# afermg/aliby

Hardware: AMD Instinct MI355X
Metric: FOV tiles/sec (whole node) (higher is better)
Workload: dtype u16 pixels, f64 feature accumulators, f32 dynamics, bfloat16 U-Net

## Files before the change

### aliby_amd/csrc/nn_conv.hip

```cpp
#include "common.h"
#include "conv_launch.h"
#include "conv_mfma.h"

namespace {

struct ConvArgs {
  const uint4* in;
  const uint4* wpk;
  uint4* out;
  uint4* pool;
  const float* scale;
  const float* shift;
  const float* bias;
  const uint4* res;
  int shift_stride, res_up;
  int cs, coff;
  int ocs, ocoff;
  int N, H, W;
  int G;
  int tiles_x, tiles_y, ntiles;
  int order;
  const uint4* pin;
  const uint4* pwpk;
  int pcs;
  const float* hscale;
  const float* hshift;
  const float* hw;
  const float* hbias;
  float* hout;
  int hO;
  const uint4* wpk2;
  const float* scale2;
  const float* shift2;
  const float* bias2;
  int shift2_stride;
  const float* fx;
  const float* fw;
  const float* fscale;
  const float* fshift;
  int fcin;
  unsigned long long* trace;
};

#define CONV_STAMP(slot_)                                                                   \
  do {                                                                                      \
    if (a.trace && blockIdx.x == 0 && tid == 0 && stamp_tile < 16)                          \
      a.trace[stamp_tile * 8 + (slot_)] = __builtin_amdgcn_s_memtime();                     \
  } while (0)



template <int R>
__device__ __forceinline__ void conv_load_res(const ConvArgs& a, int n, int irow, int row0, int gx, int c0, uint4 (&rr)[R][2]) {
  const int RH = a.H >> a.res_up, RW = a.W >> a.res_up;
  const uint4* resN = a.res + (size_t)n * RH * RW * a.ocs + a.ocoff;
#pragma unroll
  for (int r = 0; r < R; ++r) {
    const int cy = min(row0 + r, a.H - 1), cx = min(gx, a.W - 1);
    const unsigned off = (unsigned)((((irow + cy) >> a.res_up) * RW + (cx >> a.res_up)) * a.ocs + (c0 >> 3));
    rr[r][0] = resN[off];
    rr[r][1] = resN[off + 1];
  }
}

template <int R>
__device__ __forceinline__ void conv_seed(f32x16_t (&acc)[R], const float4 (&b4)[4], const uint4 (&rr)[R][2], bool has_res) {
#pragma unroll
  for (int r = 0; r < R; ++r) {
    acc_seed(acc[r], b4);
    if (has_res) {
      const unsigned rw[8] = {rr[r][0].x, rr[r][0].y, rr[r][0].z, rr[r][0].w, rr[r][1].x, rr[r][1].y, rr[r][1].z, rr[r][1].w};
#pragma unroll
      for (int q = 0; q < 8; ++q) {
        acc[r][2 * q] += cv_bf2f(rw[q] & 0xffffu);
        acc[r][2 * q + 1] += cv_bf2f(rw[q] >> 16);
      }
    }
  }
}

template <int R, int KC, int DEPTH, int PLANE, int LW, bool LOW = false>
__device__ __forceinline__ void conv_mfma(const bf16x8_t* L, const bf16x8_t (&wfrag)[9 * KC], f32x16_t (&acc)[R], const bf16x8_t* L1 = nullptr) {
  constexpr int NF = (R + 2) * 3 * KC;
  bf16x8_t ring[DEPTH];
  auto frag = [&](int f) {
    const int ir = f / (3 * KC), dx = (f / KC) % 3;
    if constexpr (LOW) return (dx == 1 ? L1 : L)[2 * (f % KC) * PLANE + ((ir + 1) >> 1) * LW + (dx == 2)];
    else return L[2 * (f % KC) * PLANE + ir * LW + dx];
  };
#pragma unroll
  for (int f = 0; f < DEPTH - 1; ++f) ring[f] = frag(f);
  static_for<NF>([&](auto fc) {
    constexpr int f = decltype(fc)::value;
    if constexpr (f + DEPTH - 1 < NF) ring[(f + DEPTH - 1) % DEPTH] = frag(f + DEPTH - 1);
    constexpr int ir = f / (3 * KC), dx = (f / KC) % 3, kc = f % KC;
    static_for<3>([&](auto dc) {
      constexpr int dy = decltype(dc)::value, r = ir - dy;
      if constexpr (r >= 0 && r < R)
        acc[r] = __builtin_amdgcn_mfma_f32_32x32x16_bf16(wfrag[(dy * 3 + dx) * KC + kc], ring[f % DEPTH], acc[r], 0, 0, 0);
    });
    __builtin_amdgcn_sched_barrier(0);
  });
}

template <int R>
__device__ __forceinline__ void conv_store(const ConvArgs& a, int n, int irow, int row0, int gx, int c0, const f32x16_t (&acc)[R]) {
  if (gx >= a.W) return;
#pragma unroll
  for (int r = 0; r < R; ++r) {
    const int gy = row0 + r;
    if (gy >= a.H) continue;
    uint4* op = a.out + (size_t)n * a.H * a.W * a.ocs + a.ocoff + (unsigned)(((irow + gy) * a.W + gx) * a.ocs + (c0 >> 3));
    acc_pack16(acc[r], op[0], op[1]);
  }
}

struct HeadW { bf16x8_t w[2]; };

__device__ __forceinline__ HeadW head_weights(const float* hw, int hO, int lane) {
  HeadW h;
  const int hh = lane >> 5, o = conv_row_channel(lane & 31);
#pragma unroll
  for (int kc = 0; kc < 2; ++kc) {
    unsigned r4[4];
#pragma unroll
    for (int j2 = 0; j2 < 4; ++j2) {
      const int c = 16 * kc + 8 * hh + 2 * j2;
      r4[j2] = cv_pack2(o < hO ? hw[o * 32 + c] : 0.f, o < hO ? hw[o * 32 + c + 1] : 0.f);
    }
    h.w[kc] = __builtin_bit_cast(bf16x8_t, make_uint4(r4[0], r4[1], r4[2], r4[3]));
  }
  return h;
}

__device__ __forceinline__ f32x16_t head_apply(uint4 lo, uint4 hi, const float* sc, const float* sh, const HeadW& hw, int hh) {
  f32x2_t s2[4], h2[4];
  const float* sp = sc + 16 * hh;
  const float* hp = sh + 16 * hh;
#pragma unroll
  for (int k = 0; k < 4; ++k) { s2[k] = f32x2_t{sp[2 * k], sp[2 * k + 1]}; h2[k] = f32x2_t{hp[2 * k], hp[2 * k + 1]}; }
  const uint4 alo = conv_act8(lo, s2, h2, 0xffffffffu);
#pragma unroll
  for (int k = 0; k < 4; ++k) { s2[k] = f32x2_t{sp[8 + 2 * k], sp[8 + 2 * k + 1]}; h2[k] = f32x2_t{hp[8 + 2 * k], hp[8 + 2 * k + 1]}; }
  const uint4 ahi = conv_act8(hi, s2, h2, 0xffffffffu);
  const uint4 send = hh ? alo : ahi;
  const uint4 recv = make_uint4(__shfl_xor(send.x, 32), __shfl_xor(send.y, 32), __shfl_xor(send.z, 32), __shfl_xor(send.w, 32));
  const uint4 b0 = hh ? recv : alo, b1 = hh ? ahi : recv;
  f32x16_t y;
#pragma unroll
  for (int k = 0; k < 16; ++k) y[k] = 0.f;
  y = __builtin_amdgcn_mfma_f32_32x32x16_bf16(hw.w[0], __builtin_bit_cast(bf16x8_t, b0), y, 0, 0, 0);
  y = __builtin_amdgcn_mfma_f32_32x32x16_bf16(hw.w[1], __builtin_bit_cast(bf16x8_t, b1), y, 0, 0, 0);
  return y;
}

__device__ __forceinline__ f32x16_t head_from_acc(const f32x16_t& acc, const float* sc, const float* sh, const HeadW& hw, int hh) {
  return head_apply(acc_pack8(acc, 0), acc_pack8(acc, 1), sc, sh, hw, hh);
}

template <int CIN, int COUT, bool TALL = false, bool PACK = false, bool HEAD = false>
struct ConvCfg {
  static constexpr int KC = CIN / 16;
  static constexpr int NPL = CIN / 8;
  static constexpr int NCB = COUT / 32;
  static constexpr int R = (CIN >= 64 || HEAD) ? 2 : 4;
  static constexpr int PASSES = (PACK && COUT >= 128) ? 7 : ((CIN >= 64 && COUT >= 64) ? 2 : 1) * (TALL ? 2 : 1) * (HEAD ? 2 : 1);
  static constexpr int RG = 4 / NCB;
  static constexpr int TH = RG * R * PASSES, TW = 32, LH = TH + 2, LW = TW + 2 + (PACK ? 1 : 0);
  static constexpr int RAW = LH * LW;
  static constexpr int PLANE = NPL == 4 ? RAW + (10 - RAW % 8) % 8 : (RAW | 1);
  static constexpr int LDS_BYTES = NPL * PLANE * 16;
  static constexpr int PIX_PER_IT = 256 / NPL;
  static constexpr int ITERS = (RAW + PIX_PER_IT - 1) / PIX_PER_IT;
  static constexpr int C3_B32T = 1;
  static constexpr int C3_B64T = 4;
  static constexpr int NBATCH = (PACK && COUT >= 128) ? 3 : (CIN >= 64 ? ((TALL && COUT == 64) ? C3_B64T : 2) : (TALL ? C3_B32T : 1));
  static constexpr int BATCH = (ITERS + NBATCH - 1) / NBATCH;
  static constexpr int DEPTH = (CIN >= 64 && COUT >= 64) ? 4 : 6;
  static constexpr int DEPTH_POOL = (CIN >= 64 && COUT >= 64) ? 3 : 6;
};

template <int CIN, int COUT, bool UP, bool POOL, int PK, bool TALL, bool PACK = false, bool HEAD = false>
__global__ __launch_bounds__(256, 2) void k_conv3x3(ConvArgs a) {
  static_assert(!PACK || (!UP && PK == 0), "packed launches: plain input, no fused projection");
  static_assert(!HEAD || (COUT == 32 && !POOL && PK == 0 && !PACK), "the fused head is built for the 32-channel last unit");
  using cfg = ConvCfg<CIN, COUT, TALL, PACK, HEAD>;
  constexpr int PPLANE = (cfg::TH * cfg::TW) | 1;
  constexpr int KC = cfg::KC, NPL = cfg::NPL, NCB = cfg::NCB, R = cfg::R, TH = cfg::TH, TW = cfg::TW;
  constexpr int LW = cfg::LW, RAW = cfg::RAW, PLANE = cfg::PLANE, PASSES = cfg::PASSES;
  constexpr int PIX_PER_IT = cfg::PIX_PER_IT, ITERS = cfg::ITERS, BATCH = cfg::BATCH;
  extern __shared__ uint4 lds[];

  const int tid = threadIdx.x, lane = tid & 63, wave = tid >> 6;
  const int cb = wave % NCB, rg = wave / NCB;
  const int px = lane & 31, hh = lane >> 5;

  bf16x8_t wfrag[9 * KC];
  {
    const bf16x8_t* wp = reinterpret_cast<const bf16x8_t*>(a.wpk) + (size_t)cb * 9 * KC * 64 + lane;
#pragma unroll
    for (int i = 0; i < 9 * KC; ++i) wfrag[i] = wp[i * 64];
  }
  bf16x8_t pfrag[PK > 0 ? PK : 1];
  if constexpr (PK > 0) {
    const bf16x8_t* pp = reinterpret_cast<const bf16x8_t*>(a.pwpk) + (size_t)cb * PK * 64 + lane;
#pragma unroll
    for (int i = 0; i < PK; ++i) pfrag[i] = pp[i * 64];
  }
  uint4* const ldsP = lds + NPL * PLANE;
  __shared__ float4 sbias[COUT / 4];
  if (tid < COUT / 4) sbias[tid] = a.bias ? reinterpret_cast<const float4*>(a.bias)[tid] : make_float4(0.f, 0.f, 0.f, 0.f);
  __shared__ float hconst[HEAD ? 2 * 32 + 4 : 1];
  HeadW hwf;
  if constexpr (HEAD) {
    hwf = head_weights(a.hw, a.hO, lane);
    if (tid < 32) {
      hconst[tid] = a.hscale[tid];
      hconst[32 + tid] = a.hshift[tid];
      if (tid < 4) hconst[64 + tid] = tid < a.hO ? a.hbias[tid] : 0.f;
    }
  }
  const int pl = tid % NPL, pix0 = tid / NPL;
  const int ly0 = pix0 / LW, lx0 = pix0 - ly0 * LW;
  f32x2_t sc[4];
#pragma unroll
  for (int k = 0; k < 4; ++k) sc[k] = f32x2_t{a.scale[pl * 8 + 2 * k], a.scale[pl * 8 + 2 * k + 1]};

  const int IH = UP ? a.H >> 1 : a.H, IW = UP ? a.W >> 1 : a.W;
  const TileWalk walk = tile_walk(a.ntiles, a.order);

  for (int stamp_tile = 0; stamp_tile < walk.count; ++stamp_tile) {
    const int tile = walk.first + stamp_tile * walk.step;
    CONV_STAMP(0);
    const int tx = tile % a.tiles_x, tyn = tile / a.tiles_x;
    const int ty = tyn % a.tiles_y, n = tyn / a.tiles_y;
    const int y0 = ty * TH, x0 = tx * TW;
    int g0 = 0, cst = x0, kb = 1 << 20, nimg = n;
    if constexpr (PACK) {
      g0 = x0 / a.W;
      cst = x0 - g0 * a.W;
      kb = a.W - cst;
      nimg = n * a.G;
    }

    f32x2_t sh[4], sh1[PACK ? 4 : 1];
    {
      const float* sp = a.shift + (size_t)(nimg + g0) * a.shift_stride + pl * 8;
#pragma unroll
      for (int k = 0; k < 4; ++k) sh[k] = f32x2_t{sp[2 * k], sp[2 * k + 1]};
      if constexpr (PACK) {
        const float* sq = a.shift + (size_t)(nimg + min(g0 + 1, a.G - 1)) * a.shift_stride + pl * 8;
#pragma unroll
        for (int k = 0; k < 4; ++k) sh1[k] = f32x2_t{sq[2 * k], sq[2 * k + 1]};
      }
    }
    const int second = (PACK && px >= kb) ? 1 : 0;
    const int gx = PACK ? (second ? px - kb : cst + px) : x0 + px;
    const int irow = PACK ? (g0 + second) * a.H : 0;
    const int c0 = cb * 32 + hh * 16;
    uint4 rr[R][2];
    auto load_res = [&](int pass) { conv_load_res<R>(a, nimg, irow, y0 + (rg * PASSES + pass) * R, gx, c0, rr); };
    if (a.res) load_res(0);
    CONV_STAMP(1);
    __syncthreads();
    CONV_STAMP(2);
    const uint4* inN = a.in + (size_t)nimg * IH * IW * a.cs + a.coff;
    int p0 = pix0, qy = ly0, qx = lx0;
    asm volatile("" : "+v"(p0), "+v"(qy), "+v"(qx));
#pragma unroll
    for (int it0 = 0; it0 < ITERS; it0 += BATCH) {
      uint4 v[BATCH];
      unsigned inside = 0, later = 0;
#pragma unroll
      for (int u = 0; u < BATCH; ++u) {
        if (it0 + u >= ITERS) break;
        int lx = qx + ((it0 + u) * PIX_PER_IT) % LW, ly = qy + ((it0 + u) * PIX_PER_IT) / LW;
        if (lx >= LW) { lx -= LW; ly += 1; }
        const int gy = y0 - 1 + ly;
        const int cy = min(max(gy, 0), a.H - 1);
        if constexpr (PACK) {
          const int gapi = kb < 32 ? kb + 1 : TW + 2;
          const int bp = lx - 1 - (lx > gapi ? 1 : 0);
          const int snd = bp >= kb ? 1 : 0;
          const int c = snd ? bp - kb : cst + bp;
          const bool ok = lx != gapi && c >= 0 && c < a.W && !(bp == TW && kb == TW) && (unsigned)gy < (unsigned)a.H;
          const int img = (snd && ok) ? g0 + 1 : g0;
          inside |= (unsigned)ok << u;
          later |= (unsigned)snd << u;
          v[u] = inN[(unsigned)(((img * a.H + cy) * IW + min(max(c, 0), a.W - 1)) * a.cs + pl)];
        } else {
          const int gxi = x0 - 1 + lx;
          inside |= (unsigned)((unsigned)gy < (unsigned)a.H && (unsigned)gxi < (unsigned)a.W) << u;
          const int cx = min(max(gxi, 0), a.W - 1);
          v[u] = inN[(unsigned)(((UP ? cy >> 1 : cy) * IW + (UP ? cx >> 1 : cx)) * a.cs + pl)];
        }
      }
#pragma unroll
      for (int u = 0; u < BATCH; ++u) {
        if (it0 + u >= ITERS) break;
        uint4 o;
        if constexpr (PACK) {
          f32x2_t shs[4];
#pragma unroll
          for (int k = 0; k < 4; ++k) shs[k] = ((later >> u) & 1u) ? sh1[k] : sh[k];
          o = conv_act8(v[u], sc, shs, 0u - ((inside >> u) & 1u));
        } else {
          o = conv_act8(v[u], sc, sh, 0u - ((inside >> u) & 1u));
        }
        if (it0 + u == ITERS - 1 && p0 + (it0 + u) * PIX_PER_IT >= RAW) continue;
        lds[pl * PLANE + p0 + (it0 + u) * PIX_PER_IT] = o;
      }
    }
    if constexpr (PK > 0) {
      constexpr int POCT = 2 * PK, PUNITS = TH * TW * POCT;
      const uint4* pN = a.pin + (size_t)n * a.H * a.W * a.pcs;
#pragma unroll
      for (int it = 0; it < (PUNITS + 255) / 256; ++it) {
        const int u = tid + it * 256;
        if (u >= PUNITS) break;
        const int oct = u % POCT, pix = u / POCT;
        const int cy = min(y0 + pix / TW, a.H - 1), cx = min(x0 + pix % TW, a.W - 1);
        uint4 v = make_uint4(0, 0, 0, 0);
        if (oct < a.pcs) v = pN[(unsigned)((cy * a.W + cx) * a.pcs + oct)];
        ldsP[oct * PPLANE + pix] = v;
      }
    }
    CONV_STAMP(3);
    __syncthreads();
    CONV_STAMP(4);

#pragma unroll
    for (int pass = 0; pass < PASSES; ++pass) {
      const int rbase = (rg * PASSES + pass) * R;
      f32x16_t acc[R];
      {
        float4 b4[4];
#pragma unroll
        for (int q = 0; q < 4; ++q) b4[q] = float4(sbias[(c0 >> 2) + q]);
        conv_seed<R>(acc, b4, rr, a.res != nullptr);
      }
      __builtin_amdgcn_sched_barrier(0);
      if (pass + 1 < PASSES && a.res) load_res(pass + 1);
      __builtin_amdgcn_sched_barrier(0);
      conv_mfma<R, KC, (POOL ? cfg::DEPTH_POOL : cfg::DEPTH), PLANE, LW>(
          reinterpret_cast<const bf16x8_t*>(lds) + hh * PLANE + rbase * LW + px + second, wfrag, acc);
      if constexpr (PK > 0) {
        const bf16x8_t* LP = reinterpret_cast<const bf16x8_t*>(ldsP) + hh * PPLANE + rbase * TW + px;
#pragma unroll
        for (int r = 0; r < R; ++r)
#pragma unroll
          for (int k = 0; k < PK; ++k)
            acc[r] = __builtin_amdgcn_mfma_f32_32x32x16_bf16(pfrag[k], LP[2 * k * PPLANE + r * TW], acc[r], 0, 0, 0);
      }
      if (pass == PASSES - 1) CONV_STAMP(5);
      if constexpr (HEAD) {
        __builtin_amdgcn_sched_barrier(0);
#pragma unroll
        for (int r = 0; r < R; ++r) {
          const f32x16_t y = head_from_acc(acc[r], hconst, hconst + 32, hwf, hh);
          const int gy = y0 + rbase + r;
          if (hh == 0 && gx < a.W && gy < a.H) {
            float* hp = a.hout + (size_t)n * a.hO * a.H * a.W + (size_t)gy * a.W + gx;
            const float yo[4] = {y[0], y[1], y[2], y[3]};
            for (int o = 0; o < a.hO; ++o) hp[(size_t)o * a.H * a.W] = yo[o] + hconst[64 + o];
          }
        }
      }
      if (!HEAD || a.out) conv_store<R>(a, nimg, irow, y0 + rbase, gx, c0, acc);
      if constexpr (POOL) {
        const int PH = a.H >> 1, PW = a.W >> 1;
#pragma unroll
        for (int r = 0; r < R; r += 2) {
          const int gy = y0 + rbase + r;
          const bool writer = (px & 1) == 0 && gx + 1 < a.W && gy + 1 < a.H;
          uint4* pp = a.pool + (size_t)nimg * PH * PW * a.ocs + a.ocoff + (unsigned)((((irow + gy) >> 1) * PW + (gx >> 1)) * a.ocs + (c0 >> 3));
#pragma unroll
          for (int half = 0; half < 2; ++half) {
            unsigned pk[4];
#pragma unroll
            for (int q = 0; q < 4; ++q) {
              const float v0 = fmaxf(acc[r][half * 8 + 2 * q], acc[r + 1][half * 8 + 2 * q]);
              const float v1 = fmaxf(acc[r][half * 8 + 2 * q + 1], acc[r + 1][half * 8 + 2 * q + 1]);
              pk[q] = cv_pack2(fmaxf(v0, __shfl_xor(v0, 1)), fmaxf(v1, __shfl_xor(v1, 1)));
            }
            if (writer) pp[half] = make_uint4(pk[0], pk[1], pk[2], pk[3]);
          }
        }
      }
    }
    CONV_STAMP(6);
  }
}

template <int CIN, int COUT, bool UP, bool PACK = false>
struct DmaCfg {
  static constexpr int KC = CIN / 16, NPL = CIN / 8, NCB = COUT / 32;
  static constexpr int WAVES_PER_SIMD = CIN >= 128 ? 1 : 2;
  static constexpr int R = CIN >= 64 ? 2 : 4;
  static constexpr int PASSES = (CIN >= 128 || COUT >= 128) ? 2 : 1;
  static constexpr int RG = 4 / NCB;
  static constexpr int TH = RG * R * PASSES, TW = 32, LH = TH + 2, LW = TW + 2 + (PACK ? 1 : 0);
  static constexpr int RAW = LH * LW;
  static constexpr int RLH = UP ? TH / 2 + 2 : LH, RLW = UP ? TW / 2 + 2 : LW;
  static constexpr bool LOWA = UP && !PACK;
  static constexpr int APIX = LOWA ? RLH * RLW : RAW;
  static constexpr int PLANE = NPL == 4 ? APIX + (10 - APIX % 8) % 8 : (APIX | 1);
  static constexpr int A_SLOTS = NPL * PLANE;
  static constexpr int PIX_PER_IT = 256 / NPL;
  static constexpr int ITERS = (APIX + PIX_PER_IT - 1) / PIX_PER_IT;
  static_assert(!LOWA || (R % 2 == 0 && 256 % NPL == 0), "LOWA: passes start on even rows; a thread activates the units it fetched");
  static constexpr int RUNITS = RLH * RLW * NPL;
  static constexpr int GIT = (RUNITS + 255) / 256;
  static constexpr int R_SLOTS = GIT * 256;
  static constexpr int LDS_BYTES = (A_SLOTS + R_SLOTS) * 16;
  static constexpr int DEPTH = (CIN >= 64 && COUT >= 64) ? 4 : 6;
};

template <int CIN, int COUT, bool UP, bool PACK = false>
__global__ __launch_bounds__(256, (DmaCfg<CIN, COUT, UP, PACK>::WAVES_PER_SIMD)) void k_conv3x3_dma(ConvArgs a) {
  static_assert(!PACK || UP, "the packed LDS-DMA variant is written for upsampled input");
  using cfg = DmaCfg<CIN, COUT, UP, PACK>;
  constexpr int KC = cfg::KC, NPL = cfg::NPL, NCB = cfg::NCB, R = cfg::R, TH = cfg::TH, TW = cfg::TW;
  constexpr int LW = cfg::LW, RAW = cfg::RAW, PLANE = cfg::PLANE, RLW = cfg::RLW, PASSES = cfg::PASSES;
  constexpr int PIX_PER_IT = cfg::PIX_PER_IT, ITERS = cfg::ITERS, GIT = cfg::GIT;
  extern __shared__ uint4 lds[];
  uint4* const ldsA = lds;
  uint4* const ldsR = lds + cfg::A_SLOTS;

  const int tid = threadIdx.x, lane = tid & 63, wave = tid >> 6;
  const int cb = wave % NCB, rg = wave / NCB;
  const int px = lane & 31, hh = lane >> 5;
  const int c0 = cb * 32 + hh * 16;

  bf16x8_t wfrag[9 * KC];
  {
    const bf16x8_t* wp = reinterpret_cast<const bf16x8_t*>(a.wpk) + (size_t)cb * 9 * KC * 64 + lane;
#pragma unroll
    for (int i = 0; i < 9 * KC; ++i) wfrag[i] = wp[i * 64];
  }
  const int pl = tid % NPL, pix0 = tid / NPL;
  const int ly0 = pix0 / LW, lx0 = pix0 - ly0 * LW;
  f32x2_t sc[4];
#pragma unroll
  for (int k = 0; k < 4; ++k) sc[k] = f32x2_t{a.scale[pl * 8 + 2 * k], a.scale[pl * 8 + 2 * k + 1]};

  const int IH = UP ? a.H >> 1 : a.H, IW = UP ? a.W >> 1 : a.W;
  const TileWalk walk = tile_walk(a.ntiles, a.order);
  const int wave_u = __builtin_amdgcn_readfirstlane(wave);

  auto issue_dma = [&](int tile) {
    const int tx = tile % a.tiles_x, tyn = tile / a.tiles_x;
    const int ty = tyn % a.tiles_y, n = tyn / a.tiles_y;
    const int ry0 = UP ? (ty * TH >> 1) - 1 : ty * TH - 1, rx0 = UP ? (tx * TW >> 1) - 1 : tx * TW - 1;
    int g0 = 0, cst = 0, half = 1 << 20;
    if constexpr (PACK) {
      g0 = (tx * TW) / a.W;
      cst = tx * TW - g0 * a.W;
      half = (a.W - cst) >> 1;
    }
    const uint4* inN = a.in + (size_t)(PACK ? n * a.G : n) * IH * IW * a.cs + a.coff;
    int t0 = tid;
    asm volatile("" : "+v"(t0));
#pragma unroll
    for (int k = 0; k < GIT; ++k) {
      const int unit = t0 + k * 256;
      const int rpix = unit / NPL, oct = unit % NPL;
      const int rly = rpix / RLW, rlx = rpix - rly * RLW;
      const int iy = min(max(ry0 + rly, 0), IH - 1);
      int ix, img = 0;
      if constexpr (PACK) {
        const bool first = rlx <= half;
        ix = min(max(first ? (cst >> 1) - 1 + rlx : rlx - half - 1, 0), IW - 1);
        img = first ? g0 : min(g0 + 1, a.G - 1);
      } else {
        ix = min(max(rx0 + rlx, 0), IW - 1);
      }
      const uint4* g = inN + (unsigned)(((img * IH + iy) * IW + ix) * a.cs + oct);
      __builtin_amdgcn_global_load_lds((const __attribute__((address_space(1))) void*)g,
                                       (__attribute__((address_space(3))) void*)(ldsR + k * 256 + wave_u * 64), 16, 0, 0);
    }
  };

  if (walk.count > 0) issue_dma(walk.first);
  for (int stamp_tile = 0; stamp_tile < walk.count; ++stamp_tile) {
    const int tile = walk.first + stamp_tile * walk.step;
    CONV_STAMP(0);
    const int tx = tile % a.tiles_x, tyn = tile / a.tiles_x;
    const int ty = tyn % a.tiles_y, n = tyn / a.tiles_y;
    const int y0 = ty * TH, x0 = tx * TW;
    int g0 = 0, cst = x0, kb = 1 << 20, nimg = n;
    if constexpr (PACK) {
      g0 = x0 / a.W;
      cst = x0 - g0 * a.W;
      kb = a.W - cst;
      nimg = n * a.G;
    }
    const int second = (PACK && px >= kb) ? 1 : 0;
    const int gx = PACK ? (second ? px - kb : cst + px) : x0 + px;
    const int irow = PACK ? (g0 + second) * a.H : 0;

    f32x2_t sh[4], sh1[PACK ? 4 : 1];
    {
      const float* sp = a.shift + (size_t)(nimg + g0) * a.shift_stride + pl * 8;
#pragma unroll
      for (int k = 0; k < 4; ++k) sh[k] = f32x2_t{sp[2 * k], sp[2 * k + 1]};
// ... 389 lines not shown
        if (i >= cfg::VALS) break;
        const int c = i / (AH * AW), rem = i - c * (AH * AW), r = rem / AW, q = rem - r * AW;
        const bool ok = (inside >> u) & 1u;
        const unsigned short b = (unsigned short)cv_f2bf(ok ? first_relu(v[u], c ? fs1 : fs0, c ? fh1 : fh0) : 0.f);
        P0h[2 * i] = b;
        if (q > 0) P0h[2 * (i - 1) + 1] = b;
        if (q == AW - 1) P0h[2 * i + 1] = 0;
        if (r >= 2 && q >= 2 && q < 2 + MW)
          rawPh[2 * ((r - 2) * MW + (q - 2)) + c] = (unsigned short)(cv_pack2(ok ? v[u] : 0.f, 0.f) & 0xffffu);
      }
      if (a.fcin < 2) {
        for (int i = tid; i < cfg::RAWP_WORDS; i += 256) rawPh[2 * i + 1] = 0;
      }
      __syncthreads();
      if (it + 1 < my_tiles) request(tile + walk.step);
      __builtin_amdgcn_sched_barrier(0);
#pragma unroll
      for (int pass = 0; pass < PASSES; ++pass) {
        const int mbase = (wave * PASSES + pass) * R;
        const int mgx = x0 - 1 + px;
#pragma unroll
        for (int r = 0; r < R; ++r) {
          const int m = mbase + r;
          f32x16_t acc;
#pragma unroll
          for (int k = 0; k < 16; ++k) acc[k] = 0.f;
#pragma unroll
          for (int kc = 0; kc < 2; ++kc) {
            const unsigned* w0 = P0 + goff[kc][0] + m * AW + px;
            const unsigned* w1 = P0 + goff[kc][1] + m * AW + px;
            const uint4 bfrag = make_uint4(w0[0] & gmask[kc][0], w0[2] & gmask[kc][0], w1[0] & gmask[kc][1], w1[2] & gmask[kc][1]);
            acc = __builtin_amdgcn_mfma_f32_32x32x16_bf16(wF[kc], __builtin_bit_cast(bf16x8_t, bfrag), acc, 0, 0, 0);
          }
          const int mgy = y0 - 1 + m;
          const unsigned keep = 0u - (unsigned)((unsigned)mgy < (unsigned)a.H && (unsigned)mgx < (unsigned)a.W);
#pragma unroll
          for (int half = 0; half < 2; ++half) {
            f32x2_t s2[4], h2[4];
            const float4* tp = reinterpret_cast<const float4*>(tabB + c0 + 8 * half);
            const float4 sa = tp[0], sb = tp[1], ha = tp[8], hb = tp[9];
            s2[0] = f32x2_t{sa.x, sa.y}; s2[1] = f32x2_t{sa.z, sa.w}; s2[2] = f32x2_t{sb.x, sb.y}; s2[3] = f32x2_t{sb.z, sb.w};
            h2[0] = f32x2_t{ha.x, ha.y}; h2[1] = f32x2_t{ha.z, ha.w}; h2[2] = f32x2_t{hb.x, hb.y}; h2[3] = f32x2_t{hb.z, hb.w};
            const uint4 raw = make_uint4(cv_pack2(acc[8 * half + 0], acc[8 * half + 1]), cv_pack2(acc[8 * half + 2], acc[8 * half + 3]),
                                         cv_pack2(acc[8 * half + 4], acc[8 * half + 5]), cv_pack2(acc[8 * half + 6], acc[8 * half + 7]));
            ldsMid[(2 * hh + half) * PLANE_MID + m * MW + px] = conv_act8(raw, s2, h2, keep);
          }
        }
      }
      __syncthreads();
    }
    __syncthreads();
    __syncthreads();
  } else {
    bf16x8_t wB[9 * KC];
    {
      const bf16x8_t* pb = reinterpret_cast<const bf16x8_t*>(a.wpk2) + lane;
#pragma unroll
      for (int i = 0; i < 9 * KC; ++i) wB[i] = pb[i * 64];
    }
    const bf16x8_t pfrag = (reinterpret_cast<const bf16x8_t*>(a.pwpk) + lane)[0];
    float4 b4[4];
    load_bias4(a.bias2, c0, b4);
    __syncthreads();
    __syncthreads();
    for (int it = 0; it < my_tiles; ++it) {
      const int tile = walk.first + it * walk.step;
      const int tx = tile % a.tiles_x, tyn = tile / a.tiles_x;
      const int ty = tyn % a.tiles_y, n = tyn / a.tiles_y;
      const int y0 = ty * TH, x0 = tx * TWO;
      const uint4* const ldsMid = ldsMid0 + (it & 1) * cfg::MID_SLOTS;
      const unsigned* const rawP = rawP0 + (it & 1) * cfg::RAWP_WORDS;
      const int gx = (px < TWO && x0 + px < a.W) ? x0 + px : a.W;
#pragma unroll
      for (int pass = 0; pass < PASSES; ++pass) {
        const int rbase = (wave * PASSES + pass) * R;
        if (rbase < TH) {
          f32x16_t acc[R];
#pragma unroll
          for (int r = 0; r < R; ++r) acc_seed(acc[r], b4);
          __builtin_amdgcn_sched_barrier(0);
          conv_mfma<R, KC, cfg::DEPTH, PLANE_MID, MW>(reinterpret_cast<const bf16x8_t*>(ldsMid) + hh * PLANE_MID + rbase * MW + px, wB, acc);
#pragma unroll
          for (int r = 0; r < R; ++r) {
            const unsigned w = hh ? 0u : rawP[(rbase + r) * MW + px];
            acc[r] = __builtin_amdgcn_mfma_f32_32x32x16_bf16(pfrag, __builtin_bit_cast(bf16x8_t, make_uint4(w, 0u, 0u, 0u)), acc[r], 0, 0, 0);
          }
          conv_store<R>(a, n, 0, y0 + rbase, gx, c0, acc);
        }
        __syncthreads();
      }
    }
  }
}

__global__ __launch_bounds__(256) void k_out_head_mfma(const uint4* __restrict__ x, const float* __restrict__ scale, const float* __restrict__ shift,
                                                       const float* __restrict__ w, const float* __restrict__ bias, int O, size_t N, size_t P,
                                                       float* __restrict__ out) {
  __shared__ float hconst[2 * 32 + 4];
  const int tid = threadIdx.x, lane = tid & 63, px = lane & 31, hh = lane >> 5;
  if (tid < 32) {
    hconst[tid] = scale[tid];
    hconst[32 + tid] = shift[tid];
    if (tid < 4) hconst[64 + tid] = tid < O ? bias[tid] : 0.f;
  }
  const HeadW hwf = head_weights(w, O, lane);
  __syncthreads();
  const size_t total = N * P, nblk = (total + 31) / 32;
  const size_t wave0 = ((size_t)blockIdx.x * blockDim.x + tid) >> 6, nwaves = ((size_t)gridDim.x * blockDim.x) >> 6;
  for (size_t b = wave0; b < nblk; b += nwaves) {
    const size_t pix = b * 32 + px;
    const bool ok = pix < total;
    const size_t q = ok ? pix : total - 1;
    const uint4 lo = x[q * 4 + 2 * hh], hi = x[q * 4 + 2 * hh + 1];
    const f32x16_t y = head_apply(lo, hi, hconst, hconst + 32, hwf, hh);
    if (ok && hh == 0) {
      const size_t n = pix / P, p = pix - n * P;
      const float yo[4] = {y[0], y[1], y[2], y[3]};
      for (int o = 0; o < O; ++o) out[(n * O + o) * P + p] = yo[o] + hconst[64 + o];
    }
  }
}

__global__ void k_pack_conv3x3(const float* w, int cout, int cin_src, int cin, int taps, unsigned short* out, size_t total) {
  const size_t i = (size_t)blockIdx.x * blockDim.x + threadIdx.x;
  if (i >= total) return;
  const int j = (int)(i & 7), lane = (int)((i >> 3) & 63);
  size_t rest = i >> 9;
  const int kcn = cin / 16;
  const int kc = (int)(rest % kcn);
  rest /= kcn;
  const int tap = (int)(rest % taps), cb = (int)(rest / taps);
  const int m = lane & 31, h = lane >> 5;
  const int co = cb * 32 + 16 * ((m >> 2) & 1) + (m & 3) + 4 * (m >> 3);
  const int ci = 16 * kc + 8 * h + j;
  float v = 0.f;
  if (ci < cin_src && co < cout) v = w[((size_t)co * cin_src + ci) * taps + tap];
  out[i] = (unsigned short)cv_f2bf(v);
}

unsigned long long* g_conv_trace = nullptr;

template <int CIN, int COUT, bool UP, bool PACK = false>
int launch_conv_dma(aliby_ctx* ctx, ConvArgs& a, hipStream_t stream) {
  using cfg = DmaCfg<CIN, COUT, UP, PACK>;
  if (const int rc = conv_tiles<cfg, PACK>(a)) return rc;
  const int cap = 32 * cfg::WAVES_PER_SIMD;
  return launch<k_conv3x3_dma<CIN, COUT, UP, PACK>, 256>(ctx, a, cfg::LDS_BYTES, cap, stream);
}

template <int CIN, int COUT, bool UP, bool TALL, bool PACK = false>
int launch_conv_reg(aliby_ctx* ctx, ConvArgs& a, hipStream_t stream) {
  using cfg = ConvCfg<CIN, COUT, TALL, PACK>;
  if (const int rc = conv_tiles<cfg, PACK>(a)) return rc;
  constexpr int PKV = PACK ? 0 : (!UP && CIN == 32 && COUT == 32) ? 1 : ((!UP && CIN == 64 && COUT == 64) ? 2 : 0);
  constexpr int P_BYTES = PKV ? 2 * PKV * ((cfg::TH * cfg::TW) | 1) * 16 : 0;
  constexpr int CAP = 64;
  if (!a.pin && !a.hout) {
    if (!a.pool) return launch<k_conv3x3<CIN, COUT, UP, false, 0, TALL, PACK>, 256>(ctx, a, cfg::LDS_BYTES, CAP, stream);
    return launch<k_conv3x3<CIN, COUT, UP, true, 0, TALL, PACK>, 256>(ctx, a, cfg::LDS_BYTES, CAP, stream);
  }
  if (a.pin) {
    if constexpr (PKV > 0) {
      ARG_CHECK(!a.pool && a.pcs >= 1 && a.pcs <= 2 * PKV, "conv3x3: fused projection: unsupported input width");
      return launch<k_conv3x3<CIN, COUT, UP, false, PKV, TALL>, 256>(ctx, a, cfg::LDS_BYTES + P_BYTES, CAP, stream);
    } else {
      aliby_set_error("conv3x3: fused projection is built for (32,32) and (64,64) without upsampling only");
      return ALIBY_ERR_UNSUPPORTED;
    }
  }
  if constexpr (COUT == 32 && CIN == 32 && !UP && !PACK) {
    ARG_CHECK(!a.pool && a.hO >= 1 && a.hO <= 3, "conv3x3: fused head: 1..3 output channels, no pooled output");
    return launch<k_conv3x3<CIN, COUT, UP, false, 0, TALL, false, true>, 256>(ctx, a, cfg::LDS_BYTES, CAP, stream);
  } else {
    aliby_set_error("conv3x3: the fused output head is built for the (32,32) unit only");
    return ALIBY_ERR_UNSUPPORTED;
  }
}

template <int CIN, int COUT, bool UP>
int launch_conv(aliby_ctx* ctx, ConvArgs& a, hipStream_t stream) {
  static const bool use_dma = env_int("ALIBY_CONV_DMA", UP) != 0;
  if (use_dma && !a.pool && !a.pin && !a.hout) {
    if constexpr (UP && COUT >= 64) {
      static const int pack_up = env_int("ALIBY_CONV_PACK", 7);
      if ((pack_up & 4) && (a.W == 56 || a.W == 112) && a.N % (224 / a.W) == 0 && a.H % DmaCfg<CIN, COUT, UP, true>::TH == 0)
        return launch_conv_dma<CIN, COUT, UP, true>(ctx, a, stream);
    }
    return launch_conv_dma<CIN, COUT, UP>(ctx, a, stream);
  }
  constexpr bool CAN_TALL = (CIN >= 64 && COUT >= 128) || (CIN == 32 && COUT == 32);
  if constexpr (!UP && COUT >= 64) {
    static const int pack_on = env_int("ALIBY_CONV_PACK", 7);
    if ((pack_on & (COUT >= 128 ? 1 : 2)) && !a.pin && (a.W == 28 || a.W == 56 || a.W == 112) && a.N % (224 / a.W) == 0 &&
        a.H % ConvCfg<CIN, COUT, false, true>::TH == 0) {
      if constexpr (CIN == 64 && COUT == 64) {
        static const bool tall64 = env_int("ALIBY_CONV_TALL64", 1) != 0;
        if (tall64 && a.H % ConvCfg<CIN, COUT, true, true>::TH == 0) return launch_conv_reg<CIN, COUT, UP, true, true>(ctx, a, stream);
      }
      return launch_conv_reg<CIN, COUT, UP, false, true>(ctx, a, stream);
    }
  }
  if (CAN_TALL && !a.pin && a.H % (2 * ConvCfg<CIN, COUT, false>::TH) == 0) return launch_conv_reg<CIN, COUT, UP, CAN_TALL>(ctx, a, stream);
  return launch_conv_reg<CIN, COUT, UP, false>(ctx, a, stream);
}

}

struct HeadArgs { const float *scale, *shift, *w, *bias; float* out; int channels; };

static int conv3x3_entry(aliby_ctx* ctx, const void* in, const void* wpk, void* out, const float* scale,
                         const float* shift, int shift_per_sample, const float* bias, const void* res,
                         int res_up, int N, int H, int W, int CIN, int COUT, int in_up,
                         int in_channels, int in_channel0, int out_channels, int out_channel0,
                         void* pool_out, const void* proj_in, const void* proj_wpk, int proj_channels, void* stream_,
                         const HeadArgs* head = nullptr) {
  hipStream_t stream = static_cast<hipStream_t>(stream_);
  ARG_CHECK(ctx && in && wpk && (out || head) && scale && shift, "conv3x3: null argument");
  ARG_CHECK(N > 0 && H > 0 && W > 0, "conv3x3: empty shape");
  ARG_CHECK(!in_up || ((H & 1) == 0 && (W & 1) == 0), "conv3x3: upsampled input needs even H, W");
  ARG_CHECK(!res || !res_up || ((H & 1) == 0 && (W & 1) == 0), "conv3x3: upsampled residual needs even H, W");
  ConvArgs a;
  a.in = static_cast<const uint4*>(in);
  a.wpk = static_cast<const uint4*>(wpk);
  a.out = static_cast<uint4*>(out);
  a.scale = scale;
  a.shift = shift;
  a.bias = bias;
  a.res = static_cast<const uint4*>(res);
  a.shift_stride = shift_per_sample == 1 ? CIN : shift_per_sample;
  a.res_up = res_up ? 1 : 0;
  a.pool = static_cast<uint4*>(pool_out);
  ARG_CHECK(!pool_out || ((H & 1) == 0 && (W & 1) == 0), "conv3x3: pooled output needs even H, W");
  if (in_channels <= 0) in_channels = CIN;
  ARG_CHECK(in_channels % 8 == 0 && in_channel0 % 8 == 0 && in_channel0 >= 0 && in_channel0 + CIN <= in_channels,
            "conv3x3: channel slice must be octet aligned and inside the input tensor");
  if (out_channels <= 0) out_channels = COUT;
  ARG_CHECK(out_channels % 8 == 0 && out_channel0 % 8 == 0 && out_channel0 >= 0 && out_channel0 + COUT <= out_channels,
            "conv3x3: output channel slice must be octet aligned and inside the output tensor");
  a.ocs = out_channels / 8;
  a.ocoff = out_channel0 / 8;
  a.trace = g_conv_trace;
  a.hscale = head ? head->scale : nullptr;
  a.hshift = head ? head->shift : nullptr;
  a.hw = head ? head->w : nullptr;
  a.hbias = head ? head->bias : nullptr;
  a.hout = head ? head->out : nullptr;
  a.hO = head ? head->channels : 0;
  a.pin = static_cast<const uint4*>(proj_in);
  a.pwpk = static_cast<const uint4*>(proj_wpk);
  a.pcs = proj_channels / 8;
  ARG_CHECK(!proj_in || (proj_wpk && proj_channels > 0 && proj_channels % 8 == 0), "conv3x3: fused projection needs packed weights and an octet-aligned width");
  a.cs = in_channels / 8;
  a.coff = in_channel0 / 8;
  a.N = N; a.H = H; a.W = W;
  if (CIN == 32 && COUT == 32 && !in_up) return launch_conv<32, 32, false>(ctx, a, stream);
  if (CIN == 64 && COUT == 32 && in_up) return launch_conv<64, 32, true>(ctx, a, stream);
  if (CIN == 64 && COUT == 64 && !in_up) return launch_conv<64, 64, false>(ctx, a, stream);
  if (CIN == 64 && COUT == 64 && in_up) return launch_conv<64, 64, true>(ctx, a, stream);
  if (CIN == 64 && COUT == 128) return in_up ? launch_conv<64, 128, true>(ctx, a, stream) : launch_conv<64, 128, false>(ctx, a, stream);
  if (CIN == 32 && COUT == 64 && !in_up) return launch_conv<32, 64, false>(ctx, a, stream);
  aliby_set_error("conv3x3: unsupported (CIN=%d, COUT=%d, upsample=%d) combination", CIN, COUT, in_up);
  return ALIBY_ERR_UNSUPPORTED;
}

extern "C" int aliby_nn_conv3x3_bf16(aliby_ctx* ctx, const void* in, const void* wpk, void* out, const float* scale,
                                     const float* shift, int shift_per_sample, const float* bias, const void* res,
                                     int res_up, int N, int H, int W, int CIN, int COUT, int in_up,
                                     int in_channels, int in_channel0, int out_channels, int out_channel0,
                                     void* pool_out, void* stream) {
  return conv3x3_entry(ctx, in, wpk, out, scale, shift, shift_per_sample, bias, res, res_up, N, H, W, CIN, COUT, in_up, in_channels,
                       in_channel0, out_channels, out_channel0, pool_out, nullptr, nullptr, 0, stream);
}

extern "C" int aliby_nn_conv3x3_proj_bf16(aliby_ctx* ctx, const void* in, const void* wpk, void* out, const float* scale,
                                          const float* shift, int shift_per_sample, const float* bias, int N, int H, int W,
                                          int CIN, int COUT, const void* proj_in, const void* proj_wpk, int proj_channels,
                                          void* stream) {
  ARG_CHECK(proj_in && proj_wpk, "conv3x3_proj: NULL projection operand");
  return conv3x3_entry(ctx, in, wpk, out, scale, shift, shift_per_sample, bias, nullptr, 0, N, H, W, CIN, COUT, 0, 0, 0, 0, 0, nullptr,
                       proj_in, proj_wpk, proj_channels, stream);
}

extern "C" int aliby_nn_conv3x3_head_bf16(aliby_ctx* ctx, const void* in, const void* wpk, void* out_or_null, const float* scale,
                                          const float* shift, int shift_per_sample, const float* bias, const void* res, int res_up,
                                          int N, int H, int W, int CIN, int COUT, const float* head_scale, const float* head_shift,
                                          const float* head_w, const float* head_bias, int head_channels, float* head_out,
                                          void* stream) {
  ARG_CHECK(head_scale && head_shift && head_w && head_bias && head_out, "conv3x3_head: NULL head operand");
  ARG_CHECK(CIN == 32 && COUT == 32, "conv3x3_head: built for the 32 -> 32 unit");
  const HeadArgs head = {head_scale, head_shift, head_w, head_bias, head_out, head_channels};
  return conv3x3_entry(ctx, in, wpk, out_or_null, scale, shift, shift_per_sample, bias, res, res_up, N, H, W, CIN, COUT, 0, 0, 0, 0, 0,
                       nullptr, nullptr, nullptr, 0, stream, &head);
}

extern "C" int aliby_nn_conv3x3_pair_bf16(aliby_ctx* ctx, const void* in, const void* wpk_a, const void* wpk_b, void* out_or_null,
                                          const float* scale_a, const float* shift_a, int shift_a_per_sample, const float* bias_a,
                                          const float* scale_b, const float* shift_b, int shift_b_per_sample, const float* bias_b,
                                          const void* res, int N, int H, int W, void* pool_out, const float* head_scale,
                                          const float* head_shift, const float* head_w, const float* head_bias, int head_channels,
                                          float* head_out, void* stream_) {
  hipStream_t stream = static_cast<hipStream_t>(stream_);
  ARG_CHECK(ctx && in && wpk_a && wpk_b && (out_or_null || head_out) && scale_a && shift_a && scale_b && shift_b, "conv3x3_pair: null argument");
  ARG_CHECK(N > 0 && H > 0 && W > 0, "conv3x3_pair: empty shape");
  ARG_CHECK(!pool_out || ((H & 1) == 0 && (W & 1) == 0), "conv3x3_pair: pooled output needs even H, W");
  ARG_CHECK(!head_out || (head_scale && head_shift && head_w && head_bias && head_channels >= 1 && head_channels <= 3 && !pool_out),
            "conv3x3_pair: the fused head needs its operands, 1..3 channels and no pooled output");
  ARG_CHECK(!pool_out || out_or_null, "conv3x3_pair: the pooled output comes with the full output");
  ConvArgs a = {};
  a.in = static_cast<const uint4*>(in);
  a.wpk = static_cast<const uint4*>(wpk_a);
  a.wpk2 = static_cast<const uint4*>(wpk_b);
  a.out = static_cast<uint4*>(out_or_null);
  a.pool = static_cast<uint4*>(pool_out);
  a.scale = scale_a; a.shift = shift_a; a.bias = bias_a;
  a.scale2 = scale_b; a.shift2 = shift_b; a.bias2 = bias_b;
  a.shift_stride = shift_a_per_sample == 1 ? 32 : shift_a_per_sample;
  a.shift2_stride = shift_b_per_sample == 1 ? 32 : shift_b_per_sample;
  a.res = static_cast<const uint4*>(res);
  a.res_up = 0;
  a.cs = 4; a.coff = 0; a.ocs = 4; a.ocoff = 0;
  a.N = N; a.H = H; a.W = W; a.G = 1;
  a.hscale = head_scale; a.hshift = head_shift; a.hw = head_w; a.hbias = head_bias; a.hout = head_out; a.hO = head_out ? head_channels : 0;
  a.tiles_x = (W + PairCfg::TWO - 1) / PairCfg::TWO;
  a.tiles_y = (H + PairCfg::TH - 1) / PairCfg::TH;
  const long long nt = (long long)N * a.tiles_x * a.tiles_y;
  ARG_CHECK(nt < INT_MAX, "conv3x3_pair: too many tiles");
  a.ntiles = (int)nt;
  constexpr int CAP = 32;
  if (!head_out && !pool_out) return launch<k_conv_pair32<false, false>, 512>(ctx, a, PairCfg::LDS_BYTES, CAP, stream);
  if (!head_out) return launch<k_conv_pair32<true, false>, 512>(ctx, a, PairCfg::LDS_BYTES, CAP, stream);
  return launch<k_conv_pair32<false, true>, 512>(ctx, a, PairCfg::LDS_BYTES, CAP, stream);
}

extern "C" int aliby_nn_first_pair_bf16(aliby_ctx* ctx, const float* tiles, int N, int Cin, int H, int W, const float* scale0,
                                        const float* shift0, const float* w_oihw, const void* wpk1, const float* scale1,
                                        const float* shift1, const float* bias1, const void* proj_wpk, void* out, void* stream_) {
  hipStream_t stream = static_cast<hipStream_t>(stream_);
  ARG_CHECK(ctx && tiles && scale0 && shift0 && w_oihw && wpk1 && scale1 && shift1 && bias1 && proj_wpk && out, "first_pair: null argument");
  ARG_CHECK(N > 0 && H > 0 && W > 0 && Cin >= 1 && Cin <= 2, "first_pair: Cin must be 1 or 2");
  ConvArgs a = {};
  a.fx = tiles; a.fw = w_oihw; a.fscale = scale0; a.fshift = shift0; a.fcin = Cin;
  a.wpk2 = static_cast<const uint4*>(wpk1);
  a.scale2 = scale1; a.shift2 = shift1; a.bias2 = bias1; a.shift2_stride = 0;
  a.pwpk = static_cast<const uint4*>(proj_wpk);
  a.out = static_cast<uint4*>(out);
  a.cs = 4; a.coff = 0; a.ocs = 4; a.ocoff = 0;
  a.N = N; a.H = H; a.W = W; a.G = 1;
  a.tiles_x = (W + FirstPairCfg::TWO - 1) / FirstPairCfg::TWO;
  a.tiles_y = (H + FirstPairCfg::TH - 1) / FirstPairCfg::TH;
  const long long nt = (long long)N * a.tiles_x * a.tiles_y;
  ARG_CHECK(nt < INT_MAX, "first_pair: too many tiles");
  a.ntiles = (int)nt;
  return launch<k_conv_first_pair, 512>(ctx, a, FirstPairCfg::LDS_BYTES, 32, stream);
}

// ... 39 lines not shown
```

Measured before the change: 631.7.

## Load fused projection operands into registers and allow packed/tall launches with projection

The fused 1x1 projection input used to be staged through an extra LDS region. It is now prefetched per pass straight into the registers that the residual prefetch used, and fed to the MFMA from there. This drops the extra LDS allocation and a shared-memory round trip. It also lets projection launches take the packed and tall tile configurations that were excluded before, at the cost of more per-lane global loads and register pressure.

```diff
diff --git a/aliby_amd/csrc/nn_conv.hip b/aliby_amd/csrc/nn_conv.hip
--- a/aliby_amd/csrc/nn_conv.hip
+++ b/aliby_amd/csrc/nn_conv.hip
@@ -63,6 +63,23 @@
   }
 }
 
+template <int R, int PK>
+__device__ __forceinline__ void conv_load_proj(const ConvArgs& a, int n, int irow, int row0, int gx, int hh, uint4 (&pf)[R][2]) {
+  static_assert(PK >= 1 && PK <= 2, "projection fragments share the registers of the residual prefetch");
+  const uint4* pN = a.pin + (size_t)n * a.H * a.W * a.pcs;
+#pragma unroll
+  for (int r = 0; r < R; ++r) {
+    const int cy = min(row0 + r, a.H - 1), cx = min(gx, a.W - 1);
+    const unsigned off = (unsigned)(((irow + cy) * a.W + cx) * a.pcs);
+#pragma unroll
+    for (int k = 0; k < PK; ++k) {
+      const int oct = 2 * k + hh;
+      const uint4 v = pN[off + min(oct, a.pcs - 1)];
+      pf[r][k] = oct < a.pcs ? v : make_uint4(0, 0, 0, 0);
+    }
+  }
+}
+
 template <int R>
 __device__ __forceinline__ void conv_seed(f32x16_t (&acc)[R], const float4 (&b4)[4], const uint4 (&rr)[R][2], bool has_res) {
 #pragma unroll
@@ -182,10 +199,9 @@
 
 template <int CIN, int COUT, bool UP, bool POOL, int PK, bool TALL, bool PACK = false, bool HEAD = false>
 __global__ __launch_bounds__(256, 2) void k_conv3x3(ConvArgs a) {
-  static_assert(!PACK || (!UP && PK == 0), "packed launches: plain input, no fused projection");
+  static_assert(!PACK || (!UP && (PK == 0 || (CIN == 64 && COUT == 64))), "packed launches: plain input; a fused projection on the 64 -> 64 unit only");
   static_assert(!HEAD || (COUT == 32 && !POOL && PK == 0 && !PACK), "the fused head is built for the 32-channel last unit");
   using cfg = ConvCfg<CIN, COUT, TALL, PACK, HEAD>;
-  constexpr int PPLANE = (cfg::TH * cfg::TW) | 1;
   constexpr int KC = cfg::KC, NPL = cfg::NPL, NCB = cfg::NCB, R = cfg::R, TH = cfg::TH, TW = cfg::TW;
   constexpr int LW = cfg::LW, RAW = cfg::RAW, PLANE = cfg::PLANE, PASSES = cfg::PASSES;
   constexpr int PIX_PER_IT = cfg::PIX_PER_IT, ITERS = cfg::ITERS, BATCH = cfg::BATCH;
@@ -207,7 +223,6 @@
 #pragma unroll
     for (int i = 0; i < PK; ++i) pfrag[i] = pp[i * 64];
   }
-  uint4* const ldsP = lds + NPL * PLANE;
   __shared__ float4 sbias[COUT / 4];
   if (tid < COUT / 4) sbias[tid] = a.bias ? reinterpret_cast<const float4*>(a.bias)[tid] : make_float4(0.f, 0.f, 0.f, 0.f);
   __shared__ float hconst[HEAD ? 2 * 32 + 4 : 1];
@@ -259,8 +274,11 @@
     const int irow = PACK ? (g0 + second) * a.H : 0;
     const int c0 = cb * 32 + hh * 16;
     uint4 rr[R][2];
-    auto load_res = [&](int pass) { conv_load_res<R>(a, nimg, irow, y0 + (rg * PASSES + pass) * R, gx, c0, rr); };
-    if (a.res) load_res(0);
+    auto load_res = [&](int pass) {
+      if constexpr (PK > 0) conv_load_proj<R, PK>(a, nimg, irow, y0 + (rg * PASSES + pass) * R, gx, hh, rr);
+      else conv_load_res<R>(a, nimg, irow, y0 + (rg * PASSES + pass) * R, gx, c0, rr);
+    };
+    if (PK == 0 && a.res) load_res(0);
     CONV_STAMP(1);
     __syncthreads();
     CONV_STAMP(2);
@@ -312,18 +330,8 @@
       }
     }
     if constexpr (PK > 0) {
-      constexpr int POCT = 2 * PK, PUNITS = TH * TW * POCT;
-      const uint4* pN = a.pin + (size_t)n * a.H * a.W * a.pcs;
-#pragma unroll
-      for (int it = 0; it < (PUNITS + 255) / 256; ++it) {
-        const int u = tid + it * 256;
-        if (u >= PUNITS) break;
-        const int oct = u % POCT, pix = u / POCT;
-        const int cy = min(y0 + pix / TW, a.H - 1), cx = min(x0 + pix % TW, a.W - 1);
-        uint4 v = make_uint4(0, 0, 0, 0);
-        if (oct < a.pcs) v = pN[(unsigned)((cy * a.W + cx) * a.pcs + oct)];
-        ldsP[oct * PPLANE + pix] = v;
-      }
+      __builtin_amdgcn_sched_barrier(0);
+      load_res(0);
     }
     CONV_STAMP(3);
     __syncthreads();
@@ -337,20 +345,22 @@
         float4 b4[4];
 #pragma unroll
         for (int q = 0; q < 4; ++q) b4[q] = float4(sbias[(c0 >> 2) + q]);
-        conv_seed<R>(acc, b4, rr, a.res != nullptr);
+        conv_seed<R>(acc, b4, rr, PK == 0 && a.res != nullptr);
       }
       __builtin_amdgcn_sched_barrier(0);
-      if (pass + 1 < PASSES && a.res) load_res(pass + 1);
+      if (PK == 0 && pass + 1 < PASSES && a.res) load_res(pass + 1);
       __builtin_amdgcn_sched_barrier(0);
       conv_mfma<R, KC, (POOL ? cfg::DEPTH_POOL : cfg::DEPTH), PLANE, LW>(
           reinterpret_cast<const bf16x8_t*>(lds) + hh * PLANE + rbase * LW + px + second, wfrag, acc);
       if constexpr (PK > 0) {
-        const bf16x8_t* LP = reinterpret_cast<const bf16x8_t*>(ldsP) + hh * PPLANE + rbase * TW + px;
 #pragma unroll
         for (int r = 0; r < R; ++r)
 #pragma unroll
           for (int k = 0; k < PK; ++k)
-            acc[r] = __builtin_amdgcn_mfma_f32_32x32x16_bf16(pfrag[k], LP[2 * k * PPLANE + r * TW], acc[r], 0, 0, 0);
+            acc[r] = __builtin_amdgcn_mfma_f32_32x32x16_bf16(pfrag[k], __builtin_bit_cast(bf16x8_t, rr[r][k]), acc[r], 0, 0, 0);
+        __builtin_amdgcn_sched_barrier(0);
+        if (pass + 1 < PASSES) load_res(pass + 1);
+        __builtin_amdgcn_sched_barrier(0);
       }
       if (pass == PASSES - 1) CONV_STAMP(5);
       if constexpr (HEAD) {
@@ -1046,8 +1056,7 @@
 int launch_conv_reg(aliby_ctx* ctx, ConvArgs& a, hipStream_t stream) {
   using cfg = ConvCfg<CIN, COUT, TALL, PACK>;
   if (const int rc = conv_tiles<cfg, PACK>(a)) return rc;
-  constexpr int PKV = PACK ? 0 : (!UP && CIN == 32 && COUT == 32) ? 1 : ((!UP && CIN == 64 && COUT == 64) ? 2 : 0);
-  constexpr int P_BYTES = PKV ? 2 * PKV * ((cfg::TH * cfg::TW) | 1) * 16 : 0;
+  constexpr int PKV = (!UP && CIN == 32 && COUT == 32) ? 1 : ((!UP && CIN == 64 && COUT == 64) ? 2 : 0);
   constexpr int CAP = 64;
   if (!a.pin && !a.hout) {
     if (!a.pool) return launch<k_conv3x3<CIN, COUT, UP, false, 0, TALL, PACK>, 256>(ctx, a, cfg::LDS_BYTES, CAP, stream);
@@ -1056,7 +1065,7 @@
   if (a.pin) {
     if constexpr (PKV > 0) {
       ARG_CHECK(!a.pool && a.pcs >= 1 && a.pcs <= 2 * PKV, "conv3x3: fused projection: unsupported input width");
-      return launch<k_conv3x3<CIN, COUT, UP, false, PKV, TALL>, 256>(ctx, a, cfg::LDS_BYTES + P_BYTES, CAP, stream);
+      return launch<k_conv3x3<CIN, COUT, UP, false, PKV, TALL, PACK>, 256>(ctx, a, cfg::LDS_BYTES, CAP, stream);
     } else {
       aliby_set_error("conv3x3: fused projection is built for (32,32) and (64,64) without upsampling only");
       return ALIBY_ERR_UNSUPPORTED;
@@ -1085,7 +1094,7 @@
   constexpr bool CAN_TALL = (CIN >= 64 && COUT >= 128) || (CIN == 32 && COUT == 32);
   if constexpr (!UP && COUT >= 64) {
     static const int pack_on = env_int("ALIBY_CONV_PACK", 7);
-    if ((pack_on & (COUT >= 128 ? 1 : 2)) && !a.pin && (a.W == 28 || a.W == 56 || a.W == 112) && a.N % (224 / a.W) == 0 &&
+    if ((pack_on & (COUT >= 128 ? 1 : 2)) && (a.W == 28 || a.W == 56 || a.W == 112) && a.N % (224 / a.W) == 0 &&
         a.H % ConvCfg<CIN, COUT, false, true>::TH == 0) {
       if constexpr (CIN == 64 && COUT == 64) {
         static const bool tall64 = env_int("ALIBY_CONV_TALL64", 1) != 0;
@@ -1094,7 +1103,7 @@
       return launch_conv_reg<CIN, COUT, UP, false, true>(ctx, a, stream);
     }
   }
-  if (CAN_TALL && !a.pin && a.H % (2 * ConvCfg<CIN, COUT, false>::TH) == 0) return launch_conv_reg<CIN, COUT, UP, CAN_TALL>(ctx, a, stream);
+  if (CAN_TALL && a.H % (2 * ConvCfg<CIN, COUT, false>::TH) == 0) return launch_conv_reg<CIN, COUT, UP, CAN_TALL>(ctx, a, stream);
   return launch_conv_reg<CIN, COUT, UP, false>(ctx, a, stream);
 }
 
```

After: 623.9. 1.2% lower.
